# agwi-lab/renderformer

Hardware: AMD Instinct MI355X
Metric: rendered frames/sec at 512×512, renderformer-v1.1-swin-large, 1/2/4/8 MI355X (higher is better)
Workload: dtype fp16+bf16

## Files before the change

renderformer_amd/csrc/gemm.hip:

```cpp
#include <algorithm>
#include <type_traits>
#include <cmath>
#include <math.h>
#include <stdio.h>
#include <stdlib.h>
#include <string.h>

#include "common.h"
#include "env.h"

namespace {

constexpr int BK = 32;
constexpr int P_F16 = 2;

enum Epi { E_BF16 = RF_EPI_BF16, E_F32 = RF_EPI_F32, E_ADD = RF_EPI_ADD_F32, E_SWIGLU = RF_EPI_SWIGLU, E_CONV = 16,
           E_ROPE = 17 };

template <int BM_, int BN_, int WGM_, int WGN_, int STAGES_, int KH_ = 1>
struct Tile {
    static constexpr int BM = BM_, BN = BN_, WGM = WGM_, WGN = WGN_, STAGES = STAGES_, KH = KH_;
    static constexpr int NWAVE = WGM * WGN, THREADS = NWAVE * 64;
    static constexpr int MW = BM / WGM, NWD = BN / WGN, TI = MW / 16, TJ = NWD / 16;
    static constexpr int APIECES = BM / 16;
// ... 2364 lines not shown
    using namespace c32;
    __shared__ __attribute__((aligned(16))) char smem[LDS];
    const int lane = threadIdx.x & 63;
    const int wave = __builtin_amdgcn_readfirstlane(threadIdx.x >> 6);
    const int nwg = gridDim.x, hw = blockIdx.x;
    const int xcd = hw & 7, q = nwg >> 3, r = nwg & 7;
    const int wg = (xcd < r ? xcd * (q + 1) : r * (q + 1) + (xcd - r) * q) + (hw >> 3);
    const int tx_n = p.wo / TW, ty_n = p.ho / TH;
    const int tx = wg % tx_n, rest = wg / tx_n;
    const int ty = rest % ty_n, img = rest / ty_n;
    const int y0 = ty * TH, x0 = tx * TW;
    const int nch = p.cin_pad / 32;

    int hpix[HPW], hch[HPW];
#pragma unroll
    for (int t = 0; t < HPW; ++t) {
        const int hp = (wave + NWAVE * t) * 16 + (lane >> 2);
        hch[t] = (lane & 3) ^ h2::hkey(hp % HWID);
        int pix = -1;
        if (hp < HPIX) {
            const int hy = hp / HWID, hx = hp - hy * HWID;
            const int iy = y0 + hy - 1, ix = x0 + hx - 1;
            if (iy >= 0 && iy < p.hi && ix >= 0 && ix < p.wi) pix = (img * p.hi + iy) * p.wi + ix;
        }
        hpix[t] = pix;
    }
    const int wr = lane >> 2;
    auto issue = [&](int chunk, int buf) {
        char* b = smem + buf * BUF;
#pragma unroll
        for (int t = 0; t < HPW; ++t) {
            const bf16_t* src = hpix[t] >= 0 ? p.a + (int64_t)hpix[t] * p.cin_pad + hch[t] * 8 + chunk * 32 : p.zero;
            __builtin_amdgcn_global_load_lds(GLB_PTR(void, src), LDS_PTR(void, b + (wave + NWAVE * t) * 1024), 16, 0, 0);
        }
        for (int v = wave; v < WPIECES; v += NWAVE) {
            const int tap = v >> 1, row = 16 * (v & 1) + wr;
            const bf16_t* src = p.w + (int64_t)row * p.ldw + tap * p.cin_pad + chunk * 32 + (((lane & 3) ^ ((row >> 1) & 3)) * 8);
            __builtin_amdgcn_global_load_lds(GLB_PTR(void, src), LDS_PTR(void, b + HBYTES + v * 1024), 16, 0, 0);
        }
    };
    const int n_issue = HPW + (WPIECES - wave + NWAVE - 1) / NWAVE;

    f32x4 acc[8][2];
#pragma unroll
    for (int i = 0; i < 8; ++i)
#pragma unroll
        for (int j = 0; j < 2; ++j) acc[i][j] = f32x4{0.f, 0.f, 0.f, 0.f};
    const int frow = lane & 15, fch = lane >> 4;
    uint32_t hadr[2][3];
#pragma unroll
    for (int h = 0; h < 2; ++h)
#pragma unroll
        for (int t = 0; t < 3; ++t) {
            const int hx = 16 * h + frow + t;
            hadr[h][t] = (uint32_t)(uintptr_t)LDS_PTR(char, smem) + ((4 * wave) * HWID + hx) * 64 +
                         ((fch ^ h2::hkey(hx)) << 4);
        }
    const uint32_t wadr = (uint32_t)(uintptr_t)LDS_PTR(char, smem) + HBYTES + lds_off(frow, fch);

    issue(0, 0);
    for (int c = 0; c < nch; ++c) {
        const int buf = c & 1;
        if (c + 1 < nch) {
            issue(c + 1, buf ^ 1);
            wait_vm_rt<16>(n_issue);
        } else {
            wait_vm<0>();
        }
        __builtin_amdgcn_s_barrier();
        __builtin_amdgcn_sched_barrier(0);
        const uint32_t bo = buf * BUF;
        bf16x8 fa[2][8], fb[2][2];
        auto rd = [&](int tap, int s) {
#pragma unroll
            for (int j = 0; j < 2; ++j)
                fb[s][j] = *LDS_PTR(const bf16x8, (uintptr_t)(wadr + bo + tap * 2048 + j * 1024));
#pragma unroll
            for (int i = 0; i < 8; ++i)
                fa[s][i] = *LDS_PTR(const bf16x8, (uintptr_t)(hadr[i & 1][tap % 3] + bo + ((i >> 1) + tap / 3) * HWID * 64));
        };
        rd(0, 0);
#pragma unroll
        for (int tap = 0; tap < 9; ++tap) {
            const int s = tap & 1;
            if (tap + 1 < 9) rd(tap + 1, s ^ 1);
            __builtin_amdgcn_sched_barrier(0);
#pragma unroll
            for (int i = 0; i < 8; ++i)
#pragma unroll
                for (int j = 0; j < 2; ++j)
                    acc[i][j] = __builtin_amdgcn_mfma_f32_16x16x32_f16(__builtin_bit_cast(f16x8, fb[s][j]),
                                                                       __builtin_bit_cast(f16x8, fa[s][i]), acc[i][j], 0, 0, 0);
            __builtin_amdgcn_sched_barrier(0);
        }
        __builtin_amdgcn_sched_barrier(0);
        __builtin_amdgcn_s_barrier();
    }

    float bsum[2][4];
#pragma unroll
    for (int j = 0; j < 2; ++j)
#pragma unroll
        for (int e = 0; e < 4; ++e) {
            const int col = j * 16 + 4 * (lane >> 4) + e;
            bsum[j][e] = (p.bias && col < p.cout) ? p.bias[col] : 0.f;
        }
    const int hwp = p.ho * p.wo;
    float sv[8][2][4];
#pragma unroll
    for (int i = 0; i < 8; ++i)
#pragma unroll
        for (int j = 0; j < 2; ++j)
#pragma unroll
            for (int e = 0; e < 4; ++e) sv[i][j][e] = silu(acc[i][j][e] + bsum[j][e]);
    const float* __restrict__ w_fin = p.w_fin;
    const float* __restrict__ b_fin = p.b_fin;
    float* __restrict__ out = reinterpret_cast<float*>(p.c);
    float wf[NFIN][2][4], bf[NFIN];
#pragma unroll
    for (int f = 0; f < NFIN; ++f) {
        bf[f] = f < p.n_fin ? b_fin[f] : 0.f;
#pragma unroll
        for (int j = 0; j < 2; ++j)
#pragma unroll
            for (int e = 0; e < 4; ++e) {
                const int col = j * 16 + 4 * (lane >> 4) + e;
                wf[f][j][e] = (f < p.n_fin && col < p.cout) ? w_fin[f * p.cout + col] : 0.f;
            }
    }
#pragma unroll
    for (int f = 0; f < NFIN; ++f) {
        if (f >= p.n_fin) break;
#pragma unroll
        for (int i = 0; i < 8; ++i) {
            float s = 0.f;
#pragma unroll
            for (int j = 0; j < 2; ++j)
#pragma unroll
                for (int e = 0; e < 4; ++e) s += sv[i][j][e] * wf[f][j][e];
            s += __shfl_xor(s, 16, 64);
            s += __shfl_xor(s, 32, 64);
            if (lane < 16) {
                const int m = (img * p.ho + y0 + 4 * wave + (i >> 1)) * p.wo + x0 + 16 * (i & 1) + lane;
                float y = elu_fast(s + bf[f], p.elu_alpha);
                if (p.flags & RF_CONV_LOG_DECODE) y = pow10m1_fast(y);
                const int64_t o = (p.flags & RF_CONV_NCHW_OUT) ? ((int64_t)(m / hwp) * p.n_fin + f) * hwp + (m % hwp)
                                                              : (int64_t)m * p.n_fin + f;
                out[o] = y;
            }
        }
    }
}

#ifdef RF_STUDY
namespace hk {
constexpr int TH = 16, TW = 32, HWID = TW + 2, HPIX = (TH + 2) * HWID;
constexpr int NCO = 64;
constexpr int HPIECES = 40, WPIECES = 9 * NCO / 16;
constexpr int HBYTES = HPIECES * 1024, WBYTES = WPIECES * 1024, BUF = HBYTES + WBYTES;
constexpr int NWAVE = 4, HPW = HPIECES / NWAVE, WPW = WPIECES / NWAVE;
constexpr int LDS = 2 * BUF;
static_assert(WPIECES % NWAVE == 0 && LDS <= 160 * 1024, "hk: LDS budget");
}
struct HkTile {
    static constexpr int WGN = 1, WGM = 4, MW = 128, NWD = 64, TI = 8, TJ = 4;
};

__global__ __launch_bounds__(256, 1) void conv3x3_hk_kernel(EngineArgs p) {
    using namespace hk;
    __shared__ __attribute__((aligned(16))) char smem[LDS];
    const int lane = threadIdx.x & 63;
    const int wave = __builtin_amdgcn_readfirstlane(threadIdx.x >> 6);
    const int nwg = gridDim.x, hw = blockIdx.x;
    const int xcd = hw & 7, q = nwg >> 3, r = nwg & 7;
    const int wg = (xcd < r ? xcd * (q + 1) : r * (q + 1) + (xcd - r) * q) + (hw >> 3);
    const int tiles_n = p.n / NCO, tx_n = p.wo / TW, ty_n = p.ho / TH;
    const int tn = wg % tiles_n, pt = wg / tiles_n;
    const int tx = pt % tx_n, rest = pt / tx_n;
    const int ty = rest % ty_n, img = rest / ty_n;
    const int y0 = ty * TH, x0 = tx * TW, n0 = tn * NCO;
    const int nch = p.cin_pad / 32;

    int hpix[HPW], hch[HPW];
#pragma unroll
    for (int t = 0; t < HPW; ++t) {
        const int hp = (wave + NWAVE * t) * 16 + (lane >> 2);
        hch[t] = (lane & 3) ^ h2::hkey(hp % HWID);
        int pix = -1;
        if (hp < HPIX) {
            const int hy = hp / HWID, hx = hp - hy * HWID;
            const int iy = y0 + hy - 1, ix = x0 + hx - 1;
            if (iy >= 0 && iy < p.hi && ix >= 0 && ix < p.wi) pix = (img * p.hi + iy) * p.wi + ix;
        }
        hpix[t] = pix;
    }
    const int wr = lane >> 2;
    const bf16_t* wsrc[WPW];
#pragma unroll
    for (int u = 0; u < WPW; ++u) {
        const int v = wave + NWAVE * u, tap = v >> 2, row = 16 * (v & 3) + wr;
        wsrc[u] = p.w + (int64_t)(n0 + row) * p.ldw + tap * p.cin_pad + (((lane & 3) ^ ((row >> 1) & 3)) * 8);
    }
    auto issue = [&](int chunk, int buf) {
        char* b = smem + buf * BUF;
#pragma unroll
        for (int t = 0; t < HPW; ++t) {
            const bf16_t* src = hpix[t] >= 0 ? p.a + (int64_t)hpix[t] * p.cin_pad + hch[t] * 8 + chunk * 32 : p.zero;
            __builtin_amdgcn_global_load_lds(GLB_PTR(void, src), LDS_PTR(void, b + (wave + NWAVE * t) * 1024), 16, 0, 0);
        }
#pragma unroll
        for (int u = 0; u < WPW; ++u)
            __builtin_amdgcn_global_load_lds(GLB_PTR(void, wsrc[u] + chunk * 32),
                                             LDS_PTR(void, b + HBYTES + (wave + NWAVE * u) * 1024), 16, 0, 0);
    };

    f32x4 acc[8][4];
#pragma unroll
    for (int i = 0; i < 8; ++i)
#pragma unroll
        for (int j = 0; j < 4; ++j) acc[i][j] = f32x4{0.f, 0.f, 0.f, 0.f};
    const int frow = lane & 15, fch = lane >> 4;
    uint32_t hadr[2][3];
#pragma unroll
    for (int h = 0; h < 2; ++h)
#pragma unroll
        for (int t = 0; t < 3; ++t) {
            const int hx = 16 * h + frow + t;
            hadr[h][t] = (uint32_t)(uintptr_t)LDS_PTR(char, smem) + ((4 * wave) * HWID + hx) * 64 +
                         ((fch ^ h2::hkey(hx)) << 4);
        }
    const uint32_t wadr = (uint32_t)(uintptr_t)LDS_PTR(char, smem) + HBYTES + lds_off(frow, fch);

    issue(0, 0);
    for (int c = 0; c < nch; ++c) {
        const int buf = c & 1;
        if (c + 1 < nch) {
            issue(c + 1, buf ^ 1);
            wait_vm<HPW + WPW>();
        } else {
            wait_vm<0>();
        }
        __builtin_amdgcn_s_barrier();
        __builtin_amdgcn_sched_barrier(0);
        const uint32_t bo = buf * BUF;
        bf16x8 fa[2][8], fb[2][4];
        auto rd = [&](int tap, int s) {
#pragma unroll
            for (int j = 0; j < 4; ++j)
                fb[s][j] = *LDS_PTR(const bf16x8, (uintptr_t)(wadr + bo + tap * 4096 + j * 1024));
#pragma unroll
            for (int i = 0; i < 8; ++i)
                fa[s][i] = *LDS_PTR(const bf16x8, (uintptr_t)(hadr[i & 1][tap % 3] + bo + ((i >> 1) + tap / 3) * HWID * 64));
        };
        rd(0, 0);
#pragma unroll
        for (int tap = 0; tap < 9; ++tap) {
            const int s = tap & 1;
            if (tap + 1 < 9) rd(tap + 1, s ^ 1);
            __builtin_amdgcn_sched_barrier(0);
#pragma unroll
            for (int i = 0; i < 8; ++i)
#pragma unroll
                for (int j = 0; j < 4; ++j)
                    acc[i][j] = __builtin_amdgcn_mfma_f32_16x16x32_f16(__builtin_bit_cast(f16x8, fb[s][j]),
                                                                       __builtin_bit_cast(f16x8, fa[s][i]), acc[i][j], 0, 0, 0);
            __builtin_amdgcn_sched_barrier(0);
        }
        __builtin_amdgcn_sched_barrier(0);
        __builtin_amdgcn_s_barrier();
    }
    engine_epilogue<HkTile, E_CONV, TW, false>(p, (img * p.ho + y0) * p.wo + x0, n0, acc);
}
#endif

using T128 = Tile<128, 128, 2, 2, 3>;
using T128w8 = Tile<128, 128, 2, 4, 3>;
using T256 = Tile<256, 256, 2, 4, 4>;
using T256x128 = Tile<256, 128, 4, 2, 3>;
using T256x64 = Tile<256, 64, 4, 1, 4>;
using T96x256 = Tile<96, 256, 2, 4, 3>;
using T64x256 = Tile<64, 256, 2, 4, 3>;
using T64x256w4 = Tile<64, 256, 1, 4, 3>;
using T96x256s5 = Tile<96, 256, 2, 4, 5>;
using T96x256s6 = Tile<96, 256, 2, 4, 6>;
using T64x256s6 = Tile<64, 256, 2, 4, 6>;
using T128s6 = Tile<128, 128, 2, 2, 6>;
using T128w8s6 = Tile<128, 128, 2, 4, 6>;
using T128k2s3 = Tile<128, 128, 2, 2, 3, 2>;
using T128k2s4 = Tile<128, 128, 2, 2, 4, 2>;
using T128w8k2s4 = Tile<128, 128, 2, 4, 4, 2>;
using T96x256k2 = Tile<96, 256, 2, 4, 3, 2>;
using T64x256k2 = Tile<64, 256, 2, 4, 3, 2>;
using T64x256w4k2 = Tile<64, 256, 1, 4, 3, 2>;
using T64c = Tile<64, 64, 2, 2, 8>;
using T64x128c = Tile<64, 128, 2, 2, 6>;

int pick_group_m(int tiles_m, int tiles_n, int bm, int bn, int64_t per_xcd, int64_t a_bytes = 0) {
    if (rf::env_set("RF_GEMM_GROUP_M")) return std::max(1, std::min(tiles_m, rf::env_int("RF_GEMM_GROUP_M", 0)));
    if (RF_ENV_ONCE("RF_GEMM_STREAM_RASTER", 1) != 0 && a_bytes > (192ll << 20) && tiles_n <= 8) return std::max(1, std::min(tiles_m, 32 / tiles_n));
    const double g = std::sqrt((double)per_xcd * bn / bm);
    int gm = (int)(g + 0.5);
    gm = std::max(1, std::min(gm, tiles_m));
    if ((int64_t)gm * tiles_n < per_xcd / 2) gm = std::min<int64_t>(tiles_m, (per_xcd + tiles_n - 1) / tiles_n);
    return gm;
}

// ... 872 lines not shown
    RF_REQUIRE(k % 128 == 0 && n % 256 == 0, "rf_gemm_mx8: K=%d must be a multiple of 128 and N=%d of 256", k, n);
    RF_REQUIRE(lda % 16 == 0 && ldw % 16 == 0 && lda >= k && ldw >= k, "rf_gemm_mx8: lda/ldw (bytes) >= K, 16-B aligned");
    RF_REQUIRE(ld_sa % 4 == 0 && ld_sw % 4 == 0 && ld_sa >= k / 32 && ld_sw >= k / 32,
               "rf_gemm_mx8: scale rows must hold K/32 bytes, 4-B aligned");
    RF_REQUIRE(((uintptr_t)a & 15) == 0 && ((uintptr_t)w & 15) == 0 && ((uintptr_t)sa & 3) == 0 && ((uintptr_t)sw & 3) == 0,
               "rf_gemm_mx8: operands 16-B / scales 4-B aligned");
    RF_REQUIRE(epilogue >= RF_EPI_BF16 && epilogue <= RF_EPI_SWIGLU, "rf_gemm_mx8: bad epilogue %d", epilogue);
    RF_REQUIRE(ldc >= (epilogue == RF_EPI_SWIGLU ? n / 2 : n) && ldc % 4 == 0, "rf_gemm_mx8: ldc too small/unaligned");
    EngineArgs p{};
    dense_args(p, a, lda, w, ldw, m, n, k, c, ldc);
    p.sa = (const uint8_t*)sa;
    p.sw = (const uint8_t*)sw;
    p.ld_sa = (int)ld_sa;
    p.ld_sw = (int)ld_sw;
    p.bias = bias;
    hipStream_t st = (hipStream_t)stream;
    if (RF_ENV_ONCE("RF_MX8_PLAIN", 0) == 0) {
        const int tiles_m = (m + 127) / 128, tiles_n = n / 256;
        const int nwg = tiles_m * tiles_n;
        p.group_m = pick_group_m(tiles_m, tiles_n, 128, 256, (nwg + 7) / 8, (int64_t)m * k);
        const dim3 g(nwg), b(512);
        return with_epi(epilogue, [&](auto e) {
            RF_LAUNCH((mx8_p3_kernel<decltype(e)::value>), g, b, 0, st, p);
            return rf::check_launch("rf_gemm_mx8");
        });
    }
    const int tiles_m = (m + 255) / 256, tiles_n = n / 256;
    const int nwg = tiles_m * tiles_n;
    p.group_m = pick_group_m(tiles_m, tiles_n, 256, 256, (nwg + 7) / 8, (int64_t)m * k);
    const dim3 g(nwg), b(512);
    return with_epi(epilogue, [&](auto e) {
        RF_LAUNCH((mx8_kernel<decltype(e)::value>), g, b, 0, st, p);
        return rf::check_launch("rf_gemm_mx8");
    });
}

extern "C" int rf_quant_mx8(const void* x, int64_t ldx, int rows, int cols, void* q, int64_t ldq, void* scales,
                            int64_t ld_s, void* stream) {
    RF_REQUIRE(x && q && scales, "rf_quant_mx8: null pointer");
    RF_REQUIRE(cols % 32 == 0 && ldx % 8 == 0 && ldq % 16 == 0 && ldq >= cols && ld_s >= cols / 32,
               "rf_quant_mx8: cols %% 32, 16-B rows");
    if (rows <= 0) return RF_OK;
    const int64_t n = (int64_t)rows * (cols / 32);
    RF_LAUNCH(quant_mx8_kernel, dim3((unsigned)((n + 255) / 256)), dim3(256), 0, (hipStream_t)stream,
                       (const bf16_t*)x, ldx, rows, cols, (uint8_t*)q, ldq, (uint8_t*)scales, ld_s);
    return rf::check_launch("rf_quant_mx8");
}

static bool halo2_ok(const EngineArgs& a) {
    const int env = rf::env_int("RF_CONV_HALO2", -1);
    if (env == 0) return false;
    if (!rf::env_set("RF_CONV_HALO2") && rf::env_set("RF_CONV_TILE")) return false;
    if (a.kw != 3 || a.k != 9 * a.cin_pad || a.stride != 1 || a.pad != 1 || a.ho != a.hi || a.wo != a.wi) return false;
    if (a.cin_pad % 32 || (a.n % 128 && a.n != 64) || a.ho % h2::TH || a.wo % h2::TW || a.m % 512) return false;
    const int64_t blocks = (int64_t)(a.m / 512) * (a.n == 64 ? 1 : a.n / 128);
    return env == 1 || blocks >= 256;
}

static int launch_halo2(EngineArgs a, void* stream, const char* what) {
    const bool n64 = a.n == 64;
    const int nwg = (a.m / 512) * (n64 ? 1 : a.n / 128);
    const int ring = rf::env_int("RF_CONV_H2S", 4);
    const hipStream_t st = (hipStream_t)stream;
    const int dbg = rf::env_int("RF_H2_DBG", 0);
#ifndef RF_STUDY
    if (dbg) return rf::study_only("rf_conv: RF_H2_DBG (halo2 ablation builds)");
#else
    if (!n64 && ring == 4 && dbg >= 1 && dbg <= 8) {
        if (dbg == 1) RF_LAUNCH((halo2_kernel<4, 128, 1>), dim3(nwg), dim3(512), 0, st, a);
        if (dbg == 2) RF_LAUNCH((halo2_kernel<4, 128, 2>), dim3(nwg), dim3(512), 0, st, a);
        if (dbg == 3) RF_LAUNCH((halo2_kernel<4, 128, 3>), dim3(nwg), dim3(512), 0, st, a);
        if (dbg == 4) RF_LAUNCH((halo2_kernel<4, 128, 4>), dim3(nwg), dim3(512), 0, st, a);
        if (dbg == 8) RF_LAUNCH((halo2_kernel<4, 128, 8>), dim3(nwg), dim3(512), 0, st, a);
        return rf::check_launch(what);
    }
#endif
    if (n64) {
        if (ring == 3) RF_LAUNCH((halo2_kernel<3, 64>), dim3(nwg), dim3(512), 0, st, a);
        else if (ring == 5) RF_LAUNCH((halo2_kernel<5, 64>), dim3(nwg), dim3(512), 0, st, a);
        else RF_LAUNCH((halo2_kernel<4, 64>), dim3(nwg), dim3(512), 0, st, a);
    } else {
        if (ring == 3) RF_LAUNCH((halo2_kernel<3, 128>), dim3(nwg), dim3(512), 0, st, a);
        else if (ring == 5) RF_LAUNCH((halo2_kernel<5, 128>), dim3(nwg), dim3(512), 0, st, a);
        else RF_LAUNCH((halo2_kernel<4, 128>), dim3(nwg), dim3(512), 0, st, a);
    }
    return rf::check_launch(what);
}

static bool halo3_ok(const EngineArgs& a) {
    if (rf::env_int("RF_CONV_HALO3", 1) == 0 || (a.flags & RF_CONV_FINAL) || a.n % 128 || a.deconv) return false;
    if ((int64_t)128 * a.ldw * 2 >= 0x7fffffff) return false;
    return halo2_ok(a);
}

static int launch_halo3(EngineArgs a, void* stream, const char* what) {
    const int nwg = (a.m / 512) * (a.n / 128);
    const int dbg = rf::env_int("RF_H3_DBG", 0);
#ifndef RF_STUDY
    if (dbg) return rf::study_only("rf_conv: RF_H3_DBG (halo3 ablation builds, garbage results)");
    RF_LAUNCH(halo3_kernel<0>, dim3(nwg), dim3(512), 0, (hipStream_t)stream, a);
#else
    if (dbg == 1) RF_LAUNCH(halo3_kernel<1>, dim3(nwg), dim3(512), 0, (hipStream_t)stream, a);
    else if (dbg == 2) RF_LAUNCH(halo3_kernel<2>, dim3(nwg), dim3(512), 0, (hipStream_t)stream, a);
    else if (dbg == 4) RF_LAUNCH(halo3_kernel<4>, dim3(nwg), dim3(512), 0, (hipStream_t)stream, a);
    else if (dbg == 6) RF_LAUNCH(halo3_kernel<6>, dim3(nwg), dim3(512), 0, (hipStream_t)stream, a);
    else if (dbg == 8) RF_LAUNCH(halo3_kernel<8>, dim3(nwg), dim3(512), 0, (hipStream_t)stream, a);
    else if (dbg == 14) RF_LAUNCH(halo3_kernel<14>, dim3(nwg), dim3(512), 0, (hipStream_t)stream, a);
    else if (dbg == 15) RF_LAUNCH(halo3_kernel<15>, dim3(nwg), dim3(512), 0, (hipStream_t)stream, a);
    else if (dbg == 30) RF_LAUNCH(halo3_kernel<30>, dim3(nwg), dim3(512), 0, (hipStream_t)stream, a);
    else if (dbg == 16) RF_LAUNCH(halo3_kernel<16>, dim3(nwg), dim3(512), 0, (hipStream_t)stream, a);
    else if (dbg == 32) RF_LAUNCH(halo3_kernel<32>, dim3(nwg), dim3(512), 0, (hipStream_t)stream, a);
    else if (dbg == 64) RF_LAUNCH(halo3_kernel<64>, dim3(nwg), dim3(512), 0, (hipStream_t)stream, a);
    else if (dbg == 96) RF_LAUNCH(halo3_kernel<96>, dim3(nwg), dim3(512), 0, (hipStream_t)stream, a);
    else RF_LAUNCH(halo3_kernel<0>, dim3(nwg), dim3(512), 0, (hipStream_t)stream, a);
#endif
    return rf::check_launch(what);
}

static bool c32_ok(const EngineArgs& a) {
    if (rf::env_int("RF_CONV_C32", 1) == 0 || !(a.flags & RF_CONV_FINAL) || a.cout > 32 || a.n < 32) return false;
    if (a.kw != 3 || a.k != 9 * a.cin_pad || a.stride != 1 || a.pad != 1 || a.ho != a.hi || a.wo != a.wi) return false;
    return a.cin_pad % 32 == 0 && a.ho % c32::TH == 0 && a.wo % c32::TW == 0 && a.m > 0 && a.n_fin <= c32::NFIN;
}

static int launch_c32(EngineArgs a, void* stream, const char* what) {
    const int nwg = a.m / (c32::TH * c32::TW);
    RF_LAUNCH(conv3x3_c32_kernel, dim3(nwg), dim3(256), 0, (hipStream_t)stream, a);
    return rf::check_launch(what);
}

static bool hk_ok(const EngineArgs& a) {
    const int env = rf::env_int("RF_CONV_HK", 0);
    if (env == 0 || (a.flags & RF_CONV_FINAL) || a.deconv) return false;
#ifndef RF_STUDY
    return true;
#else
    if (a.kw != 3 || a.k != 9 * a.cin_pad || a.stride != 1 || a.pad != 1 || a.ho != a.hi || a.wo != a.wi) return false;
    if (a.cin_pad % 32 || a.n % hk::NCO || a.ho % hk::TH || a.wo % hk::TW || a.m <= 0) return false;
    return env == 1 || (int64_t)(a.m / (hk::TH * hk::TW)) * (a.n / hk::NCO) >= 256;
#endif
}

static int launch_hk(EngineArgs a, void* stream, const char* what) {
#ifdef RF_STUDY
    const int nwg = (a.m / (hk::TH * hk::TW)) * (a.n / hk::NCO);
    RF_LAUNCH(conv3x3_hk_kernel, dim3(nwg), dim3(256), 0, (hipStream_t)stream, a);
    return rf::check_launch(what);
#else
    (void)a, (void)stream, (void)what;
    return rf::study_only("rf_conv: RF_CONV_HK=1 (conv3x3_hk_kernel)");
#endif
}

enum ConvTile : int {
    CT_AUTO = 0,
    CT_64 = 64,
    CT_128 = 128,
    CT_256 = 256,
    CT_128w8 = 1288,
    CT_256x128 = 2561,
    CT_64x128 = 6412,
    CT_64SK = 6464,
};
static int conv_tile_env() { return rf::env_int("RF_CONV_TILE", CT_AUTO); }

template <bool GATHER>
static int conv_f16_dp(EngineArgs& p, void* stream, const char* what, int tile = 0) {
    if (GATHER && c32_ok(p)) return launch_c32(p, stream, what);
    if (GATHER && hk_ok(p)) return launch_hk(p, stream, what);
    if (GATHER && halo3_ok(p)) return launch_halo3(p, stream, what);
    if (GATHER && halo2_ok(p)) return launch_halo2(p, stream, what);
    const int t = tile ? tile : conv_tile_env();
    if (p.n == 64) return launch_conv<T256x64, P_F16, GATHER>(p, stream, what);
    if (t == CT_64 || t == CT_64SK) return launch_conv<T64c, P_F16, GATHER>(p, stream, what);
    if (t == CT_64x128) return launch_conv<T64x128c, P_F16, GATHER>(p, stream, what);
    if (t == CT_128) return launch_conv<T128, P_F16, GATHER>(p, stream, what);
    if (t == CT_128w8) return launch_conv<T128w8, P_F16, GATHER>(p, stream, what);
    if (t == CT_256x128) return launch<T256x128, E_CONV, P_F16, GATHER>(p, stream, what);
    if (p.n % 256 == 0 && (t == CT_256 || (t == CT_AUTO && ((p.m + 255) / 256) * (p.n / 256) >= 256)))
        return (rf::env_int("RF_CONV_PHASED", 0) != 0 && use_phased(p.n, p.k))
                   ? launch_phased<E_CONV, P_F16, GATHER, 256>(p, stream, what)
                   : launch_conv<T256, P_F16, GATHER>(p, stream, what);
    const int64_t tiles = (int64_t)((p.m + 127) / 128) * (p.n / 128);
    if (tiles <= 512) return launch_conv<T128w8, P_F16, GATHER>(p, stream, what);
    return launch_conv<T128, P_F16, GATHER>(p, stream, what);
}

template <int NT>
static int conv_dispatch(EngineArgs& p, bool gather, bool big, int64_t sk_grid_n, void* workspace, void* stream,
                         const char* what, int tile = 0) {
    if constexpr (NT == P_F16) {
        if (!sk_grid_n)
            return gather ? conv_f16_dp<true>(p, stream, what, tile) : conv_f16_dp<false>(p, stream, what, tile);
    }
    if (sk_grid_n) {
        if (const int rc = sk_setup(p, workspace, stream)) return rc;
        if (NT == P_F16 && rf::env_int("RF_CONV_SKW8", 1) != 0)
            return gather ? launch_sk<T128w8, E_CONV, NT, true>(p, (int)sk_grid_n, stream, what)
                          : launch_sk<T128w8, E_CONV, NT, false>(p, (int)sk_grid_n, stream, what);
        return gather ? launch_sk<T128, E_CONV, NT, true>(p, (int)sk_grid_n, stream, what)
                      : launch_sk<T128, E_CONV, NT, false>(p, (int)sk_grid_n, stream, what);
    }
    if (gather)
        return big ? launch<T256x128, E_CONV, NT, true>(p, stream, what) : launch<T128, E_CONV, NT, true>(p, stream, what);
    return big ? launch<T256x128, E_CONV, NT, false>(p, stream, what) : launch<T128, E_CONV, NT, false>(p, stream, what);
}

static int conv_common(EngineArgs& p, int nterm, bool gather, const void* w_hi, const void* w_lo, int cout, int cout_pad, float* out,
                       const float* bias, const float* res1, const float* res2, void* p_hi, void* p_lo, int p_ld,
                       int flags, const float* w_fin, const float* b_fin, int n_fin, float elu_alpha, void* workspace,
                       int64_t ws_bytes, void* stream, const char* what) {
    RF_REQUIRE(w_hi && (w_lo || nterm == P_F16), "%s: null weights", what);
    RF_REQUIRE(cout % 4 == 0, "%s: cout must be a multiple of 4", what);
    RF_REQUIRE(out || p_hi, "%s: no output", what);
    RF_REQUIRE(!p_hi || ((p_lo || nterm == P_F16) && p_ld % 4 == 0 && p_ld >= cout), "%s: bad plane output", what);
    RF_REQUIRE(!(flags & RF_CONV_FINAL) || (cout <= 64 && w_fin && b_fin && n_fin > 0 && out),
               "%s: final head needs cout <= 64 and w_fin/b_fin", what);
    RF_REQUIRE(!(flags & RF_CONV_BORDER_BIAS) ||
                   (bias && !(flags & RF_CONV_FINAL) && p.kw == 3 && p.k == 9 * p.cin_pad && p.stride == 1 &&
                    p.pad == 1 && p.ho == p.hi && p.wo == p.wi && p.deconv == 0 && p.ho >= 2 && p.wo >= 2),
               "%s: RF_CONV_BORDER_BIAS needs a 3x3 stride-1 pad-1 convolution of an image of at least 2 x 2 pixels "
               "with its 9-row bias", what);
    static void* z = nullptr;
    if (!z && hipGetSymbolAddress(&z, HIP_SYMBOL(g_zero_row)) != hipSuccess) {
        z = nullptr;
        rf::set_error("%s: zero row symbol", what);
        return RF_ERR_LAUNCH;
    }
    p.zero = (const bf16_t*)z;
    p.w = (const bf16_t*)w_hi;
    p.w_lo = (const bf16_t*)w_lo;
    p.n = cout_pad;
    p.c = out;
    p.bias = bias;
    p.res1 = res1;
    p.res2 = res2;
    p.p_hi = (bf16_t*)p_hi;
    p.p_lo = (bf16_t*)p_lo;
    p.p_ld = p_ld;
    p.plane_f16 = nterm == P_F16;
    p.range = (p_hi && nterm == P_F16) ? rf::range_word() : nullptr;
    p.cout = cout;
    p.flags = flags;
    p.w_fin = w_fin;
    p.b_fin = b_fin;
    p.n_fin = n_fin;
    p.elu_alpha = elu_alpha;
    if (p.m <= 0) return RF_OK;
    const bool big = rf::env_set("RF_CONV_TILE") ? conv_tile_env() == CT_256 : ((p.m + 255) / 256) * (p.n / 128) >= 256;
    int64_t skg = 0;
    int ct = conv_tile_env();
    if (!ct && RF_ENV_ONCE("RF_CONV_SMALL", 1) != 0 && nterm == P_F16 && gather && p.kw == 3 && p.n % 64 == 0 && p.m <= 4096 &&
        (p.k <= 2304 || p.m <= 1024))
        ct = p.k <= 2304 ? CT_64 : CT_64SK;
    if (nterm == P_F16 && ct == CT_64SK && p.n % 64 == 0 && workspace && ws_bytes >= SK_WS_BYTES) {
        const int64_t tiles = (int64_t)((p.m + 63) / 64) * (p.n / 64);
        const int64_t grid = std::min<int64_t>(512, tiles * (p.k / BK) / 12);
        if (grid > tiles) {
            if (const int rc = sk_setup(p, workspace, stream)) return rc;
            return gather ? launch_sk<T64c, E_CONV, P_F16, true>(p, (int)grid, stream, what)
                          : launch_sk<T64c, E_CONV, P_F16, false>(p, (int)grid, stream, what);
        }
    }
    if (!big && p.n % 128 == 0 && workspace && ws_bytes >= SK_WS_BYTES && rf::env_int("RF_CONV_SK", 1) != 0 &&
        !(nterm == P_F16 && (ct == CT_64 || ct == CT_64x128 || ct == CT_64SK))) {
        const int64_t tiles = (int64_t)((p.m + 127) / 128) * (p.n / 128);
        const int64_t work = tiles * (p.k / BK);
        const int64_t grid = std::min<int64_t>(256, work / 8);
        if (tiles < 192 && grid > tiles) skg = grid;
    }
    return nterm == P_F16 ? conv_dispatch<P_F16>(p, gather, big, skg, workspace, stream, what, ct == CT_64 ? CT_64 : CT_AUTO)
                          : conv_dispatch<3>(p, gather, big, skg, workspace, stream, what);
}

extern "C" int rf_conv2d_bf16x3(const void* in_hi, const void* in_lo, int n_img, int hi, int wi, int cin_pad,
                                const void* w_hi, const void* w_lo, int cout, int cout_pad, int kh, int kw, int stride,
                                int pad, const float* bias, const float* res1, const float* res2, float* out,
                                void* p_hi, void* p_lo, int p_ld, int flags, const float* w_fin, const float* b_fin,
                                int n_fin, float elu_alpha, void* workspace, int64_t ws_bytes, void* stream) {
    RF_REQUIRE(in_hi && in_lo, "rf_conv2d_bf16x3: null input");
    RF_REQUIRE(cin_pad % BK == 0, "rf_conv2d_bf16x3: cin_pad %d must be a multiple of %d", cin_pad, BK);
    RF_REQUIRE(cout_pad % 128 == 0 && cout_pad >= cout, "rf_conv2d_bf16x3: cout_pad %d must be a multiple of 128",
               cout_pad);
    EngineArgs p{};
    p.a = (const bf16_t*)in_hi;
    p.a_lo = (const bf16_t*)in_lo;
    p.hi = hi;
    p.wi = wi;
    p.cin_pad = cin_pad;
    p.cin_m = udiv_magic(cin_pad);
    p.ho = (hi + 2 * pad - kh) / stride + 1;
    p.wo = (wi + 2 * pad - kw) / stride + 1;
    p.kw = kw;
    p.kw_m = udiv_magic(kw);
    p.stride = stride;
    p.pad = pad;
    p.m = n_img * p.ho * p.wo;
    p.k = kh * kw * cin_pad;
    RF_REQUIRE(p.k < 65536, "conv: kh*kw*cin_pad = %d must be < 65536", p.k);
    p.ldw = p.k;
    return conv_common(p, 3, true, w_hi, w_lo, cout, cout_pad, out, bias, res1, res2, p_hi, p_lo, p_ld, flags, w_fin,
                       b_fin, n_fin, elu_alpha, workspace, ws_bytes, stream, "rf_conv2d_bf16x3");
}

extern "C" int rf_conv2d_f16(const void* in, int n_img, int hi, int wi, int cin_pad, const void* w, int cout,
                             int cout_pad, int kh, int kw, int stride, int pad, const float* bias, const float* res1,
                             const float* res2, float* out, void* p_out, int p_ld, int flags, const float* w_fin,
                             const float* b_fin, int n_fin, float elu_alpha, void* workspace, int64_t ws_bytes,
                             void* stream) {
    RF_REQUIRE(in, "rf_conv2d_f16: null input");
    RF_REQUIRE(cin_pad % BK == 0, "rf_conv2d_f16: cin_pad %d must be a multiple of %d", cin_pad, BK);
    RF_REQUIRE((cout_pad % 128 == 0 || cout_pad == 64) && cout_pad >= cout,
               "rf_conv2d_f16: cout_pad %d must be 64 or a multiple of 128", cout_pad);
    EngineArgs p{};
    p.a = (const bf16_t*)in;
    p.hi = hi;
    p.wi = wi;
    p.cin_pad = cin_pad;
    p.cin_m = udiv_magic(cin_pad);
    p.ho = (hi + 2 * pad - kh) / stride + 1;
    p.wo = (wi + 2 * pad - kw) / stride + 1;
    p.kw = kw;
    p.kw_m = udiv_magic(kw);
    p.stride = stride;
    p.pad = pad;
    p.m = n_img * p.ho * p.wo;
    p.k = kh * kw * cin_pad;
    RF_REQUIRE(p.k < 65536, "conv: kh*kw*cin_pad = %d must be < 65536", p.k);
    p.ldw = p.k;
    return conv_common(p, P_F16, true, w, nullptr, cout, cout_pad, out, bias, res1, res2, p_out, nullptr, p_ld, flags,
                       w_fin, b_fin, n_fin, elu_alpha, workspace, ws_bytes, stream, "rf_conv2d_f16");
}

static const char* group_member(EngineArgs& p, const rf_conv_desc& d, const void* zero) {
    if (!d.in || !d.w || !(d.out || d.p_out)) return "null pointer";
    if (d.cin_pad % BK) return "cin_pad must be a multiple of 32";
    if (d.cout % 4) return "cout must be a multiple of 4";
    if (d.p_out && (d.p_ld % 4 || d.p_ld < d.cout)) return "bad p_ld";
    if (d.flags & RF_CONV_FINAL) return "the fused final head runs on its own launch";
    p = EngineArgs{};
    p.a = (const bf16_t*)d.in;
    p.cin_pad = d.cin_pad;
    p.cin_m = udiv_magic(d.cin_pad);
    p.zero = (const bf16_t*)zero;
    if (d.deconv_k > 0) {
        p.hi = p.ho = d.hi;
        p.wi = p.wo = d.wi;
        p.kw = 1;
        p.stride = 1;
        p.pad = 0;
        p.deconv = d.deconv_k;
        p.n = d.deconv_k * d.deconv_k * d.cout;
        if (d.flags) return "a deconvolution takes no flags";
    } else {
        p.hi = d.hi;
        p.wi = d.wi;
        p.ho = (d.hi + 2 * d.pad - d.kh) / d.stride + 1;
        p.wo = (d.wi + 2 * d.pad - d.kw) / d.stride + 1;
        p.kw = d.kw;
        p.stride = d.stride;
        p.pad = d.pad;
        p.n = d.cout_pad;
        if (d.cout_pad < d.cout) return "cout_pad < cout";
        if ((d.flags & RF_CONV_BORDER_BIAS) &&
            !(d.bias && d.kh == 3 && d.kw == 3 && d.stride == 1 && d.pad == 1 && d.hi >= 2 && d.wi >= 2))
            return "RF_CONV_BORDER_BIAS needs a 3x3 stride-1 pad-1 convolution of an image of at least 2 x 2 pixels "
                   "with its 9-row bias";
    }
    p.kw_m = udiv_magic(p.kw);
    p.m = d.n_img * p.ho * p.wo;
    p.k = (d.deconv_k > 0 ? 1 : d.kh * d.kw) * d.cin_pad;
    if (p.k >= 65536) return "kh*kw*cin_pad must be < 65536";
    if (p.n % T128w8::BN) return "output channels (k*k*cout for a deconvolution) must be a multiple of 128";
    p.ldw = p.k;
    p.w = (const bf16_t*)d.w;
    p.c = d.out;
    p.bias = d.bias;
    p.p_hi = (bf16_t*)d.p_out;
    p.p_ld = d.p_ld;
    p.plane_f16 = 1;
    p.range = d.p_out ? rf::range_word() : nullptr;
    p.cout = d.cout;
    p.flags = d.flags;
    return nullptr;
}

template <bool DENSE>
static int conv_group_launch(int n_conv, const rf_conv_desc* convs, void* stream, const char* what) {
    RF_REQUIRE(n_conv >= 1 && n_conv <= GROUP_MAX && convs, "%s: 1..%d convolutions", what, GROUP_MAX);
    static void* z = nullptr;
    if (!z && hipGetSymbolAddress(&z, HIP_SYMBOL(g_zero_row)) != hipSuccess) {
        z = nullptr;
        rf::set_error("%s: zero row symbol", what);
        return RF_ERR_LAUNCH;
    }
    using C = std::conditional_t<DENSE, T128w8k2s4, T128w8>;
    GroupArgs g{};
    g.n = n_conv;
    int blocks = 0;
    for (int q = 0; q < n_conv; ++q) {
        const char* err = group_member(g.p[q], convs[q], z);
        RF_REQUIRE(!err, "%s: conv %d: %s", what, q, err ? err : "");
        EngineArgs& p = g.p[q];
        if constexpr (DENSE) {
// ... 86 lines not shown
```

Measured before the change: 95.91.

## Add halo-tiled small-geometry 3x3 conv kernel with auto geometry selection

Adds a templated halo-tile implicit-GEMM 3x3 conv kernel (several spatial tile and output-channel block sizes) that loads an input halo once into LDS and reuses it across all nine taps, double-buffered over channel chunks. A picker chooses the largest geometry that still yields enough workgroups and routes small or odd-shaped fp16 convs there instead of the generic gather/split-K paths. This is meant to cut redundant global loads for convs that the existing halo kernels reject. It adds more template instantiations and may underfill the GPU for very small layers.

```diff
diff --git a/renderformer_amd/csrc/gemm.hip b/renderformer_amd/csrc/gemm.hip
--- a/renderformer_amd/csrc/gemm.hip
+++ b/renderformer_amd/csrc/gemm.hip
@@ -2540,6 +2540,131 @@
     }
 }
 
+template <int TH_, int TW_, int BN_>
+struct HsCfg {
+    static constexpr int TH = TH_, TW = TW_, BN = BN_, NWAVE = 4;
+    static constexpr int HWID = TW + 2, HPIX = (TH + 2) * HWID;
+    static constexpr int HPW = ((HPIX + 15) / 16 + NWAVE - 1) / NWAVE, HPIECES = HPW * NWAVE;
+    static constexpr int WPIECES = 9 * BN / 16, WPW = (WPIECES + NWAVE - 1) / NWAVE;
+    static constexpr int HBYTES = HPIECES * 1024, WBYTES = WPIECES * 1024, BUF = HBYTES + WBYTES, LDS = 2 * BUF;
+    static constexpr int RW = TH / NWAVE, FX = TW / 16, TI = RW * FX, TJ = BN / 16;
+    static_assert(TH % NWAVE == 0 && TW % 16 == 0 && BN % 16 == 0, "hs: whole fragments per wave");
+    static_assert(HPW + WPW <= 24 && LDS <= 160 * 1024, "hs: vmcnt range, LDS budget");
+};
+template <class G>
+struct HsTile {
+    static constexpr int WGN = 1, WGM = G::NWAVE, MW = G::RW * G::TW, NWD = G::BN, TI = G::TI, TJ = G::TJ;
+};
+
+template <int TH_, int TW_, int BN_>
+__global__ __launch_bounds__(256, 1) void conv3x3_hs_kernel(EngineArgs p, int tiles_n) {
+    using G = HsCfg<TH_, TW_, BN_>;
+    constexpr int TH = G::TH, TW = G::TW, HWID = G::HWID, HPIX = G::HPIX, NWAVE = G::NWAVE, HPW = G::HPW,
+                  WPIECES = G::WPIECES, WPW = G::WPW, HBYTES = G::HBYTES, BUF = G::BUF, TI = G::TI, TJ = G::TJ,
+                  FX = G::FX;
+    __shared__ __attribute__((aligned(16))) char smem[G::LDS];
+    const int lane = threadIdx.x & 63;
+    const int wave = __builtin_amdgcn_readfirstlane(threadIdx.x >> 6);
+    const int nwg = gridDim.x, hw = blockIdx.x;
+    const int xcd = hw & 7, q = nwg >> 3, r = nwg & 7;
+    const int wg = (xcd < r ? xcd * (q + 1) : r * (q + 1) + (xcd - r) * q) + (hw >> 3);
+    const int tx_n = p.wo / TW, ty_n = p.ho / TH;
+    const int tn = wg % tiles_n, pt = wg / tiles_n;
+    const int tx = pt % tx_n, rest = pt / tx_n;
+    const int ty = rest % ty_n, img = rest / ty_n;
+    const int y0 = ty * TH, x0 = tx * TW, n0 = tn * G::BN;
+    const int nch = p.cin_pad / 32;
+
+    int hpix[HPW], hch[HPW];
+#pragma unroll
+    for (int t = 0; t < HPW; ++t) {
+        const int hp = (wave + NWAVE * t) * 16 + (lane >> 2);
+        hch[t] = (lane & 3) ^ h2::hkey(hp % HWID);
+        int pix = -1;
+        if (hp < HPIX) {
+            const int hy = hp / HWID, hx = hp - hy * HWID;
+            const int iy = y0 + hy - 1, ix = x0 + hx - 1;
+            if (iy >= 0 && iy < p.hi && ix >= 0 && ix < p.wi) pix = (img * p.hi + iy) * p.wi + ix;
+        }
+        hpix[t] = pix;
+    }
+    const int wr = lane >> 2;
+    auto issue = [&](int chunk, int buf) {
+        char* b = smem + buf * BUF;
+#pragma unroll
+        for (int t = 0; t < HPW; ++t) {
+            const bf16_t* src = hpix[t] >= 0 ? p.a + (int64_t)hpix[t] * p.cin_pad + hch[t] * 8 + chunk * 32 : p.zero;
+            __builtin_amdgcn_global_load_lds(GLB_PTR(void, src), LDS_PTR(void, b + (wave + NWAVE * t) * 1024), 16, 0, 0);
+        }
+#pragma unroll
+        for (int u = 0; u < WPW; ++u) {
+            const int v = wave + NWAVE * u;
+            if (WPIECES % NWAVE != 0 && v >= WPIECES) break;
+            const int tap = v / TJ, row = 16 * (v % TJ) + wr;
+            const bf16_t* src = p.w + (int64_t)(n0 + row) * p.ldw + tap * p.cin_pad + chunk * 32 + (((lane & 3) ^ ((row >> 1) & 3)) * 8);
+            __builtin_amdgcn_global_load_lds(GLB_PTR(void, src), LDS_PTR(void, b + HBYTES + v * 1024), 16, 0, 0);
+        }
+    };
+    const int n_issue = HPW + (WPIECES - wave + NWAVE - 1) / NWAVE;
+
+    f32x4 acc[TI][TJ];
+#pragma unroll
+    for (int i = 0; i < TI; ++i)
+#pragma unroll
+        for (int j = 0; j < TJ; ++j) acc[i][j] = f32x4{0.f, 0.f, 0.f, 0.f};
+    const int frow = lane & 15, fch = lane >> 4;
+    uint32_t hadr[FX][3];
+#pragma unroll
+    for (int h = 0; h < FX; ++h)
+#pragma unroll
+        for (int t = 0; t < 3; ++t) {
+            const int hx = 16 * h + frow + t;
+            hadr[h][t] = (uint32_t)(uintptr_t)LDS_PTR(char, smem) + ((G::RW * wave) * HWID + hx) * 64 +
+                         ((fch ^ h2::hkey(hx)) << 4);
+        }
+    const uint32_t wadr = (uint32_t)(uintptr_t)LDS_PTR(char, smem) + HBYTES + lds_off(frow, fch);
+
+    issue(0, 0);
+    for (int c = 0; c < nch; ++c) {
+        const int buf = c & 1;
+        if (c + 1 < nch) {
+            issue(c + 1, buf ^ 1);
+            wait_vm_rt<HPW + WPW>(n_issue);
+        } else {
+            wait_vm<0>();
+        }
+        __builtin_amdgcn_s_barrier();
+        __builtin_amdgcn_sched_barrier(0);
+        const uint32_t bo = buf * BUF;
+        bf16x8 fa[2][TI], fb[2][TJ];
+        auto rd = [&](int tap, int s) {
+#pragma unroll
+            for (int j = 0; j < TJ; ++j)
+                fb[s][j] = *LDS_PTR(const bf16x8, (uintptr_t)(wadr + bo + (tap * TJ + j) * 1024));
+#pragma unroll
+            for (int i = 0; i < TI; ++i)
+                fa[s][i] = *LDS_PTR(const bf16x8, (uintptr_t)(hadr[i % FX][tap % 3] + bo + (i / FX + tap / 3) * HWID * 64));
+        };
+        rd(0, 0);
+#pragma unroll
+        for (int tap = 0; tap < 9; ++tap) {
+            const int s = tap & 1;
+            if (tap + 1 < 9) rd(tap + 1, s ^ 1);
+            __builtin_amdgcn_sched_barrier(0);
+#pragma unroll
+            for (int i = 0; i < TI; ++i)
+#pragma unroll
+                for (int j = 0; j < TJ; ++j)
+                    acc[i][j] = __builtin_amdgcn_mfma_f32_16x16x32_f16(__builtin_bit_cast(f16x8, fb[s][j]),
+                                                                       __builtin_bit_cast(f16x8, fa[s][i]), acc[i][j], 0, 0, 0);
+            __builtin_amdgcn_sched_barrier(0);
+        }
+        __builtin_amdgcn_sched_barrier(0);
+        __builtin_amdgcn_s_barrier();
+    }
+    engine_epilogue<HsTile<G>, E_CONV, TW, false>(p, (img * p.ho + y0) * p.wo + x0, n0, acc);
+}
+
 #ifdef RF_STUDY
 namespace hk {
 constexpr int TH = 16, TW = 32, HWID = TW + 2, HPIX = (TH + 2) * HWID;
@@ -3718,6 +3843,54 @@
 #endif
 }
 
+enum HsGeom : int { HS_NONE = 0, HS_16x32x64 = 163264, HS_16x32x32 = 163232, HS_8x16x64 = 81664, HS_8x16x32 = 81632 };
+struct HsChoice {
+    int code, th, tw, bn;
+};
+static constexpr HsChoice HS_GEOMS[] = {
+    {HS_16x32x64, 16, 32, 64}, {HS_16x32x32, 16, 32, 32}, {HS_8x16x64, 8, 16, 64}, {HS_8x16x32, 8, 16, 32}};
+static int64_t hs_blocks(const EngineArgs& a, const HsChoice& g) {
+    if (a.ho % g.th || a.wo % g.tw || a.cout % g.bn) return 0;
+    return (int64_t)(a.m / (g.th * g.tw)) * (a.cout / g.bn);
+}
+static int hs_pick(const EngineArgs& a) {
+    const int env = rf::env_int("RF_CONV_HALO_SMALL", 1);
+    if (env == 0 || (a.flags & RF_CONV_FINAL) || a.deconv || a.m <= 0) return HS_NONE;
+    if (!rf::env_set("RF_CONV_HALO_SMALL") && rf::env_set("RF_CONV_TILE")) return HS_NONE;
+    if (a.kw != 3 || a.k != 9 * a.cin_pad || a.stride != 1 || a.pad != 1 || a.ho != a.hi || a.wo != a.wi) return HS_NONE;
+    if (a.cin_pad % 32 || a.cout % 32 || a.cout > a.n) return HS_NONE;
+    if (a.ho % h2::TH == 0 && a.wo % h2::TW == 0 && (a.n % 128 == 0 || a.n == 64) &&
+        (int64_t)(a.m / 512) * (a.n == 64 ? 1 : a.n / 128) >= 256)
+        return HS_NONE;
+    if (env != 1) {
+        for (const HsChoice& g : HS_GEOMS)
+            if (g.code == env) return hs_blocks(a, g) ? g.code : HS_NONE;
+        return HS_NONE;
+    }
+    int code = HS_NONE;
+    for (const HsChoice& g : HS_GEOMS) {
+        const int64_t blocks = hs_blocks(a, g);
+        if (blocks) code = g.code;
+        if (blocks >= 256) break;
+    }
+    return code;
+}
+
+template <int TH, int TW, int BN>
+static int launch_hs_t(const EngineArgs& a, void* stream, const char* what) {
+    const int tiles_n = a.cout / BN;
+    const int nwg = (a.m / (TH * TW)) * tiles_n;
+    RF_LAUNCH((conv3x3_hs_kernel<TH, TW, BN>), dim3(nwg), dim3(256), 0, (hipStream_t)stream, a, tiles_n);
+    return rf::check_launch(what);
+}
+
+static int launch_hs(const EngineArgs& a, int code, void* stream, const char* what) {
+    if (code == HS_16x32x64) return launch_hs_t<16, 32, 64>(a, stream, what);
+    if (code == HS_16x32x32) return launch_hs_t<16, 32, 32>(a, stream, what);
+    if (code == HS_8x16x64) return launch_hs_t<8, 16, 64>(a, stream, what);
+    return launch_hs_t<8, 16, 32>(a, stream, what);
+}
+
 enum ConvTile : int {
     CT_AUTO = 0,
     CT_64 = 64,
@@ -3816,6 +3989,9 @@
     const bool big = rf::env_set("RF_CONV_TILE") ? conv_tile_env() == CT_256 : ((p.m + 255) / 256) * (p.n / 128) >= 256;
     int64_t skg = 0;
     int ct = conv_tile_env();
+    if (nterm == P_F16 && gather && !hk_ok(p) && !halo3_ok(p) && !halo2_ok(p)) {
+        if (const int hs = hs_pick(p)) return launch_hs(p, hs, stream, what);
+    }
     if (!ct && RF_ENV_ONCE("RF_CONV_SMALL", 1) != 0 && nterm == P_F16 && gather && p.kw == 3 && p.n % 64 == 0 && p.m <= 4096 &&
         (p.k <= 2304 || p.m <= 1024))
         ct = p.k <= 2304 ? CT_64 : CT_64SK;
```

After: 97.44 (median of 6 runs). 1.6% higher.
